# raywan-110/AdaQP

Hardware: NVIDIA H100
Metric: epochs_per_sec (higher is better)
Workload: dtype f32

## Files before the change

adaqp_b200/csrc/gemm.cu:

```cuda
#include <cuda.h>

#include "common.cuh"

namespace {

constexpr int kGemmThreads = 384;
constexpr int kBlockM = 128;
constexpr int kMaxN = 256;

__device__ __forceinline__ uint32_t smem_addr(const void *p) { return (uint32_t)__cvta_generic_to_shared(p); }

__device__ __forceinline__ void mbar_init(uint32_t bar, uint32_t count) {
    asm volatile("mbarrier.init.shared::cta.b64 [%0], %1;" ::"r"(bar), "r"(count) : "memory");
}
__device__ __forceinline__ void mbar_expect_tx(uint32_t bar, uint32_t bytes) {
    asm volatile("mbarrier.arrive.expect_tx.shared::cta.b64 _, [%0], %1;" ::"r"(bar), "r"(bytes) : "memory");
}
__device__ __forceinline__ void mbar_arrive(uint32_t bar) {
    asm volatile("mbarrier.arrive.shared::cta.b64 _, [%0];" ::"r"(bar) : "memory");
}
__device__ __forceinline__ void mbar_wait(uint32_t bar, uint32_t parity) {
    uint32_t done = 0;
    for (uint32_t spin = 0; spin < (1u << 26); ++spin) {
        asm volatile(
            "{\n"
            ".reg .pred p;\n"
            "mbarrier.try_wait.parity.shared::cta.b64 p, [%1], %2;\n"
            "selp.u32 %0, 1, 0, p;\n"
            "}\n" : "=r"(done) : "r"(bar), "r"(parity) : "memory");
        if (done) return;
    }
    __trap();
}
__device__ __forceinline__ void tma_load_2d(uint32_t dst, const CUtensorMap *map, int c0, int c1, uint32_t bar) {
    asm volatile("cp.async.bulk.tensor.2d.shared::cluster.global.tile.mbarrier::complete_tx::bytes [%0], [%1, {%2, %3}], [%4];"
                 ::"r"(dst), "l"(map), "r"(c0), "r"(c1), "r"(bar) : "memory");
}
__device__ __forceinline__ void wgmma_fence() { asm volatile("wgmma.fence.sync.aligned;" ::: "memory"); }
__device__ __forceinline__ void wgmma_commit() { asm volatile("wgmma.commit_group.sync.aligned;" ::: "memory"); }
__device__ __forceinline__ void wgmma_wait_all() { asm volatile("wgmma.wait_group.sync.aligned 0;" ::: "memory"); }

__device__ __forceinline__ uint64_t wgmma_desc(uint32_t saddr, uint32_t row_bytes) {
    uint64_t d = 0;
    d |= (uint64_t)((saddr >> 4) & 0x3FFF);
    d |= (uint64_t)1 << 16;
    d |= (uint64_t)((8u * row_bytes) >> 4) << 32;
    d |= (uint64_t)(row_bytes == 128 ? 1 : 2) << 62;
    return d;
}

__device__ __forceinline__ uint32_t swizzled(uint32_t r, uint32_t c, uint32_t row_bytes) {
    const uint32_t o = r * row_bytes + c * 4u;
    return o ^ (((o >> 7) & (row_bytes == 128 ? 7u : 3u)) << 4);
}

__device__ __forceinline__ void split_tf32(float x, uint32_t &hi, uint32_t &lo) {
    const float h = __uint_as_float(__float_as_uint(x) & 0xFFFFE000u);
    hi = __float_as_uint(h);
    lo = __float_as_uint(x - h);
}

template <int N> struct Wgmma;
template <> struct Wgmma<64> {
    static __device__ __forceinline__ void mma(float (&d)[32], const uint32_t (&a)[4], uint64_t b, uint32_t acc) {
        asm volatile(
            "{\n.reg .pred p;\nsetp.ne.b32 p, %37, 0;\n"
            "wgmma.mma_async.sync.aligned.m64n64k8.f32.tf32.tf32 {"
            "%0, %1, %2, %3, %4, %5, %6, %7, %8, %9, %10, %11, %12, %13, %14, %15, "
            "%16, %17, %18, %19, %20, %21, %22, %23, %24, %25, %26, %27, %28, %29, %30, %31"
            "}, {%32, %33, %34, %35}, %36, p, 1, 1;\n}\n"
            : "+f"(d[0]), "+f"(d[1]), "+f"(d[2]), "+f"(d[3]), "+f"(d[4]), "+f"(d[5]), "+f"(d[6]), "+f"(d[7]),
              "+f"(d[8]), "+f"(d[9]), "+f"(d[10]), "+f"(d[11]), "+f"(d[12]), "+f"(d[13]), "+f"(d[14]), "+f"(d[15]),
              "+f"(d[16]), "+f"(d[17]), "+f"(d[18]), "+f"(d[19]), "+f"(d[20]), "+f"(d[21]), "+f"(d[22]), "+f"(d[23]),
              "+f"(d[24]), "+f"(d[25]), "+f"(d[26]), "+f"(d[27]), "+f"(d[28]), "+f"(d[29]), "+f"(d[30]), "+f"(d[31])
            : "r"(a[0]), "r"(a[1]), "r"(a[2]), "r"(a[3]), "l"(b), "r"(acc));
    }
};
template <> struct Wgmma<128> {
    static __device__ __forceinline__ void mma(float (&d)[64], const uint32_t (&a)[4], uint64_t b, uint32_t acc) {
        asm volatile(
            "{\n.reg .pred p;\nsetp.ne.b32 p, %69, 0;\n"
            "wgmma.mma_async.sync.aligned.m64n128k8.f32.tf32.tf32 {"
            "%0, %1, %2, %3, %4, %5, %6, %7, %8, %9, %10, %11, %12, %13, %14, %15, "
            "%16, %17, %18, %19, %20, %21, %22, %23, %24, %25, %26, %27, %28, %29, %30, %31, "
            "%32, %33, %34, %35, %36, %37, %38, %39, %40, %41, %42, %43, %44, %45, %46, %47, "
            "%48, %49, %50, %51, %52, %53, %54, %55, %56, %57, %58, %59, %60, %61, %62, %63"
            "}, {%64, %65, %66, %67}, %68, p, 1, 1;\n}\n"
            : "+f"(d[0]), "+f"(d[1]), "+f"(d[2]), "+f"(d[3]), "+f"(d[4]), "+f"(d[5]), "+f"(d[6]), "+f"(d[7]),
              "+f"(d[8]), "+f"(d[9]), "+f"(d[10]), "+f"(d[11]), "+f"(d[12]), "+f"(d[13]), "+f"(d[14]), "+f"(d[15]),
              "+f"(d[16]), "+f"(d[17]), "+f"(d[18]), "+f"(d[19]), "+f"(d[20]), "+f"(d[21]), "+f"(d[22]), "+f"(d[23]),
              "+f"(d[24]), "+f"(d[25]), "+f"(d[26]), "+f"(d[27]), "+f"(d[28]), "+f"(d[29]), "+f"(d[30]), "+f"(d[31]),
              "+f"(d[32]), "+f"(d[33]), "+f"(d[34]), "+f"(d[35]), "+f"(d[36]), "+f"(d[37]), "+f"(d[38]), "+f"(d[39]),
              "+f"(d[40]), "+f"(d[41]), "+f"(d[42]), "+f"(d[43]), "+f"(d[44]), "+f"(d[45]), "+f"(d[46]), "+f"(d[47]),
              "+f"(d[48]), "+f"(d[49]), "+f"(d[50]), "+f"(d[51]), "+f"(d[52]), "+f"(d[53]), "+f"(d[54]), "+f"(d[55]),
              "+f"(d[56]), "+f"(d[57]), "+f"(d[58]), "+f"(d[59]), "+f"(d[60]), "+f"(d[61]), "+f"(d[62]), "+f"(d[63])
            : "r"(a[0]), "r"(a[1]), "r"(a[2]), "r"(a[3]), "l"(b), "r"(acc));
    }
};
template <> struct Wgmma<256> {
    static __device__ __forceinline__ void mma(float (&d)[128], const uint32_t (&a)[4], uint64_t b, uint32_t acc) {
        asm volatile(
            "{\n.reg .pred p;\nsetp.ne.b32 p, %133, 0;\n"
            "wgmma.mma_async.sync.aligned.m64n256k8.f32.tf32.tf32 {"
            "%0, %1, %2, %3, %4, %5, %6, %7, %8, %9, %10, %11, %12, %13, %14, %15, "
            "%16, %17, %18, %19, %20, %21, %22, %23, %24, %25, %26, %27, %28, %29, %30, %31, "
            "%32, %33, %34, %35, %36, %37, %38, %39, %40, %41, %42, %43, %44, %45, %46, %47, "
            "%48, %49, %50, %51, %52, %53, %54, %55, %56, %57, %58, %59, %60, %61, %62, %63, "
            "%64, %65, %66, %67, %68, %69, %70, %71, %72, %73, %74, %75, %76, %77, %78, %79, "
            "%80, %81, %82, %83, %84, %85, %86, %87, %88, %89, %90, %91, %92, %93, %94, %95, "
            "%96, %97, %98, %99, %100, %101, %102, %103, %104, %105, %106, %107, %108, %109, %110, %111, "
            "%112, %113, %114, %115, %116, %117, %118, %119, %120, %121, %122, %123, %124, %125, %126, %127"
            "}, {%128, %129, %130, %131}, %132, p, 1, 1;\n}\n"
            : "+f"(d[0]), "+f"(d[1]), "+f"(d[2]), "+f"(d[3]), "+f"(d[4]), "+f"(d[5]), "+f"(d[6]), "+f"(d[7]),
              "+f"(d[8]), "+f"(d[9]), "+f"(d[10]), "+f"(d[11]), "+f"(d[12]), "+f"(d[13]), "+f"(d[14]), "+f"(d[15]),
              "+f"(d[16]), "+f"(d[17]), "+f"(d[18]), "+f"(d[19]), "+f"(d[20]), "+f"(d[21]), "+f"(d[22]), "+f"(d[23]),
              "+f"(d[24]), "+f"(d[25]), "+f"(d[26]), "+f"(d[27]), "+f"(d[28]), "+f"(d[29]), "+f"(d[30]), "+f"(d[31]),
              "+f"(d[32]), "+f"(d[33]), "+f"(d[34]), "+f"(d[35]), "+f"(d[36]), "+f"(d[37]), "+f"(d[38]), "+f"(d[39]),
              "+f"(d[40]), "+f"(d[41]), "+f"(d[42]), "+f"(d[43]), "+f"(d[44]), "+f"(d[45]), "+f"(d[46]), "+f"(d[47]),
              "+f"(d[48]), "+f"(d[49]), "+f"(d[50]), "+f"(d[51]), "+f"(d[52]), "+f"(d[53]), "+f"(d[54]), "+f"(d[55]),
              "+f"(d[56]), "+f"(d[57]), "+f"(d[58]), "+f"(d[59]), "+f"(d[60]), "+f"(d[61]), "+f"(d[62]), "+f"(d[63]),
              "+f"(d[64]), "+f"(d[65]), "+f"(d[66]), "+f"(d[67]), "+f"(d[68]), "+f"(d[69]), "+f"(d[70]), "+f"(d[71]),
              "+f"(d[72]), "+f"(d[73]), "+f"(d[74]), "+f"(d[75]), "+f"(d[76]), "+f"(d[77]), "+f"(d[78]), "+f"(d[79]),
              "+f"(d[80]), "+f"(d[81]), "+f"(d[82]), "+f"(d[83]), "+f"(d[84]), "+f"(d[85]), "+f"(d[86]), "+f"(d[87]),
              "+f"(d[88]), "+f"(d[89]), "+f"(d[90]), "+f"(d[91]), "+f"(d[92]), "+f"(d[93]), "+f"(d[94]), "+f"(d[95]),
              "+f"(d[96]), "+f"(d[97]), "+f"(d[98]), "+f"(d[99]), "+f"(d[100]), "+f"(d[101]), "+f"(d[102]), "+f"(d[103]),
              "+f"(d[104]), "+f"(d[105]), "+f"(d[106]), "+f"(d[107]), "+f"(d[108]), "+f"(d[109]), "+f"(d[110]), "+f"(d[111]),
              "+f"(d[112]), "+f"(d[113]), "+f"(d[114]), "+f"(d[115]), "+f"(d[116]), "+f"(d[117]), "+f"(d[118]), "+f"(d[119]),
              "+f"(d[120]), "+f"(d[121]), "+f"(d[122]), "+f"(d[123]), "+f"(d[124]), "+f"(d[125]), "+f"(d[126]), "+f"(d[127])
            : "r"(a[0]), "r"(a[1]), "r"(a[2]), "r"(a[3]), "l"(b), "r"(acc));
    }
};

__device__ __forceinline__ void load_split_a(const uint8_t *tile, uint32_t row_bytes, int r, int c, uint32_t (&hi)[4],
                                             uint32_t (&lo)[4]) {
    split_tf32(*reinterpret_cast<const float *>(tile + swizzled(r, c, row_bytes)), hi[0], lo[0]);
    split_tf32(*reinterpret_cast<const float *>(tile + swizzled(r + 8, c, row_bytes)), hi[1], lo[1]);
    split_tf32(*reinterpret_cast<const float *>(tile + swizzled(r, c + 4, row_bytes)), hi[2], lo[2]);
    split_tf32(*reinterpret_cast<const float *>(tile + swizzled(r + 8, c + 4, row_bytes)), hi[3], lo[3]);
}

template <int KB>
struct GemmCfg {
    static constexpr int kStages = KB == 32 ? 2 : 4;
    static constexpr uint32_t kRowBytes = KB * 4;
    static constexpr uint32_t kATile = kBlockM * KB * 4;
    static constexpr uint32_t kBTile = kMaxN * KB * 4;
    static constexpr uint32_t kStageBytes = kATile + 2 * kBTile;
    static constexpr uint32_t kSmemBytes = kStages * kStageBytes + 1024 + 256;
};

template <int KB, int NM>
__global__ void __launch_bounds__(kGemmThreads, 1)
gemm_tf32x3_kernel(const __grid_constant__ CUtensorMap map_a, const __grid_constant__ CUtensorMap map_bhi,
                   const __grid_constant__ CUtensorMap map_blo, const float *__restrict__ bias,
                   float *__restrict__ C, int64_t ldc, int M, int N, int K) {
    using Cfg = GemmCfg<KB>;
    constexpr int kStages = Cfg::kStages;
    extern __shared__ uint8_t smem_raw[];
    const uint32_t base = (smem_addr(smem_raw) + 1023u) & ~1023u;
    const uint8_t *gen = smem_raw + (base - smem_addr(smem_raw));
    const uint32_t bars = base + kStages * Cfg::kStageBytes;
    auto bar_full = [&](int s) { return bars + 8u * s; };
    auto bar_empty = [&](int s) { return bars + 8u * (kStages + s); };

    const int wg = threadIdx.x >> 7;
    const int k_blocks = (K + KB - 1) / KB;
    const int tiles = (M + kBlockM - 1) / kBlockM;
    const uint32_t stage_tx = Cfg::kATile + 2u * (uint32_t)NM * KB * 4u;

    if (threadIdx.x == 0) {
        for (int s = 0; s < kStages; ++s) { mbar_init(bar_full(s), 1); mbar_init(bar_empty(s), 8); }
        asm volatile("fence.mbarrier_init.release.cluster;" ::: "memory");
    }
    __syncthreads();

    if (wg == 0) {
        if (threadIdx.x == 0) {
            int s = 0; uint32_t ph = 0;
            for (int t = blockIdx.x; t < tiles; t += gridDim.x) {
                for (int kb = 0; kb < k_blocks; ++kb) {
                    mbar_wait(bar_empty(s), ph ^ 1u);
                    const uint32_t st = base + s * Cfg::kStageBytes;
                    mbar_expect_tx(bar_full(s), stage_tx);
                    tma_load_2d(st, &map_a, kb * KB, t * kBlockM, bar_full(s));
                    tma_load_2d(st + Cfg::kATile, &map_bhi, kb * KB, 0, bar_full(s));
                    tma_load_2d(st + Cfg::kATile + Cfg::kBTile, &map_blo, kb * KB, 0, bar_full(s));
                    if (++s == kStages) { s = 0; ph ^= 1u; }
                }
            }
        }
        return;
    }
    const int tid = threadIdx.x - 128 * wg;
    const int warp = tid >> 5, lane = tid & 31, g = lane >> 2, q = lane & 3;
    const int r0 = (wg - 1) * 64 + warp * 16 + g;
    const bool vec2 = (ldc & 1) == 0 && (reinterpret_cast<uintptr_t>(C) & 7) == 0;
    float acc[NM / 2];
#pragma unroll
    for (int i = 0; i < NM / 2; ++i) acc[i] = 0.f;
    int s = 0; uint32_t ph = 0;
    for (int t = blockIdx.x; t < tiles; t += gridDim.x) {
        for (int kb = 0; kb < k_blocks; ++kb) {
            mbar_wait(bar_full(s), ph);
            const uint8_t *ta = gen + s * Cfg::kStageBytes;
            const uint32_t bhi = base + s * Cfg::kStageBytes + Cfg::kATile, blo = bhi + Cfg::kBTile;
#pragma unroll
            for (int k = 0; k < KB / 8; ++k) {
                uint32_t ahi[4], alo[4];
                load_split_a(ta, Cfg::kRowBytes, r0, k * 8 + q, ahi, alo);
                const uint64_t dhi = wgmma_desc(bhi + k * 32, Cfg::kRowBytes), dlo = wgmma_desc(blo + k * 32, Cfg::kRowBytes);
                wgmma_fence();
                Wgmma<NM>::mma(acc, alo, dhi, (kb | k) != 0);
                Wgmma<NM>::mma(acc, ahi, dlo, 1);
                Wgmma<NM>::mma(acc, ahi, dhi, 1);
                wgmma_commit();
                wgmma_wait_all();
            }
            __syncwarp();
            if (lane == 0) mbar_arrive(bar_empty(s));
            if (++s == kStages) { s = 0; ph ^= 1u; }
        }
#pragma unroll
        for (int j = 0; j < NM / 8; ++j) {
            const int col = j * 8 + 2 * q;
            const float b0 = (bias && col < N) ? __ldg(bias + col) : 0.f;
            const float b1 = (bias && col + 1 < N) ? __ldg(bias + col + 1) : 0.f;
#pragma unroll
            for (int h = 0; h < 2; ++h) {
                const int64_t row = (int64_t)t * kBlockM + r0 + 8 * h;
                if (row < M && col < N) {
                    float *p = C + row * ldc + col;
                    const float v0 = bias ? acc[4 * j + 2 * h] + b0 : acc[4 * j + 2 * h];
                    const float v1 = bias ? acc[4 * j + 2 * h + 1] + b1 : acc[4 * j + 2 * h + 1];
                    if (vec2 && col + 1 < N) {
                        *reinterpret_cast<float2 *>(p) = make_float2(v0, v1);
                    } else {
                        p[0] = v0;
                        if (col + 1 < N) p[1] = v1;
                    }
                }
            }
        }
    }
}

constexpr int kWgThreads = 384;
constexpr int kWgRows = 32;
constexpr int kWgStages = 3;
constexpr int kWgTileN = 128;
constexpr uint32_t kWgBox = kWgRows * 128;
constexpr uint32_t kWgDy = 4 * kWgBox;
constexpr uint32_t kWgX = 8 * kWgBox;
constexpr uint32_t kWgStageBytes = kWgDy + kWgX;
constexpr uint32_t kWgXt = kMaxN * 128;
constexpr uint32_t kWgSmemBytes = kWgStages * kWgStageBytes + 2 * kWgXt + 1024 + 256;

__device__ __forceinline__ void consumers_sync() { asm volatile("bar.sync 1, 256;" ::: "memory"); }

template <int NM>
__global__ void __launch_bounds__(kWgThreads, 1)
wgrad_tf32x3_kernel(const __grid_constant__ CUtensorMap map_dy, const __grid_constant__ CUtensorMap map_x,
                    float *__restrict__ partials, int M, int N, int K) {
    extern __shared__ uint8_t smem_raw[];
    const uint32_t base = (smem_addr(smem_raw) + 1023u) & ~1023u;
    uint8_t *gen = smem_raw + (base - smem_addr(smem_raw));
    const uint32_t xt_hi = base + kWgStages * kWgStageBytes, xt_lo = xt_hi + kWgXt;
    const uint32_t bars = xt_lo + kWgXt;
    auto bar_full = [&](int s) { return bars + 8u * s; };
    auto bar_empty = [&](int s) { return bars + 8u * (kWgStages + s); };

    const int wg = threadIdx.x >> 7;
    const int n0 = blockIdx.y * kWgTileN;
    const int n_left = (N - n0 + 31) / 32;
    const int n_chunks = n_left < 4 ? n_left : 4;
    const int k_chunks = (K + 31) / 32;
    const int blocks = (M + kWgRows - 1) / kWgRows;
    const int per = (blocks + gridDim.x - 1) / gridDim.x;
    const int b0 = blockIdx.x * per;
    const int b1 = (b0 + per < blocks) ? b0 + per : blocks;
    const uint32_t stage_tx = (uint32_t)(n_chunks + k_chunks) * kWgBox;

    if (threadIdx.x == 0) {
        for (int s = 0; s < kWgStages; ++s) { mbar_init(bar_full(s), 1); mbar_init(bar_empty(s), 8); }
        asm volatile("fence.mbarrier_init.release.cluster;" ::: "memory");
    }
    __syncthreads();

    if (wg == 0) {
        if (threadIdx.x == 0) {
            int s = 0; uint32_t ph = 0;
            for (int b = b0; b < b1; ++b) {
                mbar_wait(bar_empty(s), ph ^ 1u);
                const uint32_t st = base + s * kWgStageBytes;
                mbar_expect_tx(bar_full(s), stage_tx);
                for (int c = 0; c < n_chunks; ++c) tma_load_2d(st + c * kWgBox, &map_dy, n0 + c * 32, b * kWgRows, bar_full(s));
                for (int c = 0; c < k_chunks; ++c) tma_load_2d(st + kWgDy + c * kWgBox, &map_x, c * 32, b * kWgRows, bar_full(s));
                if (++s == kWgStages) { s = 0; ph ^= 1u; }
            }
        }
        return;
    }
    const int ctid = threadIdx.x - 128;
    const int tid = threadIdx.x - 128 * wg;
    const int warp = tid >> 5, lane = tid & 31, g = lane >> 2, q = lane & 3;
    const int nr = (wg - 1) * 64 + warp * 16 + g;
    const bool active = n0 + (wg - 1) * 64 < N;
    float acc[NM / 2];
#pragma unroll
    for (int i = 0; i < NM / 2; ++i) acc[i] = 0.f;
    int s = 0; uint32_t ph = 0;
    for (int b = b0; b < b1; ++b) {
        mbar_wait(bar_full(s), ph);
        const uint8_t *st = gen + s * kWgStageBytes;
        consumers_sync();
        for (int idx = ctid; idx < NM * kWgRows; idx += 256) {
            const int j = idx % NM, m = idx / NM;
            const float v = j < 32 * k_chunks
                ? *reinterpret_cast<const float *>(st + kWgDy + (j >> 5) * kWgBox + m * 128 + (j & 31) * 4) : 0.f;
            uint32_t h, l;
            split_tf32(v, h, l);
            const uint32_t o = swizzled(j, m, 128);
            *reinterpret_cast<uint32_t *>(gen + (xt_hi - base) + o) = h;
            *reinterpret_cast<uint32_t *>(gen + (xt_lo - base) + o) = l;
        }
        asm volatile("fence.proxy.async.shared::cta;" ::: "memory");
        consumers_sync();
        if (active) {
#pragma unroll
            for (int k = 0; k < kWgRows / 8; ++k) {
                uint32_t ahi[4], alo[4];
#pragma unroll
                for (int i = 0; i < 4; ++i) {
                    const int n = nr + 8 * (i & 1), m = 8 * k + q + 4 * (i >> 1);
                    split_tf32(*reinterpret_cast<const float *>(st + (n >> 5) * kWgBox + swizzled(m, n & 31, 128)), ahi[i], alo[i]);
                }
                const uint64_t dhi = wgmma_desc(xt_hi + k * 32, 128), dlo = wgmma_desc(xt_lo + k * 32, 128);
                wgmma_fence();
                Wgmma<NM>::mma(acc, alo, dhi, (b != b0) || (k != 0));
                Wgmma<NM>::mma(acc, ahi, dlo, 1);
                Wgmma<NM>::mma(acc, ahi, dhi, 1);
                wgmma_commit();
                wgmma_wait_all();
            }
        }
        __syncwarp();
        if (lane == 0) mbar_arrive(bar_empty(s));
        if (++s == kWgStages) { s = 0; ph ^= 1u; }
    }
    float *out = partials + (size_t)blockIdx.x * N * K;
#pragma unroll
    for (int j = 0; j < NM / 8; ++j) {
#pragma unroll
        for (int h = 0; h < 2; ++h) {
            const int n = n0 + nr + 8 * h;
#pragma unroll
            for (int e = 0; e < 2; ++e) {
                const int col = j * 8 + 2 * q + e;
                if (n < N && col < K) out[(size_t)n * K + col] = acc[4 * j + 2 * h + e];
            }
        }
    }
}

typedef CUresult (*EncodeTiledFn)(CUtensorMap *, CUtensorMapDataType, cuuint32_t, void *, const cuuint64_t *, const cuuint64_t *,
                                  const cuuint32_t *, const cuuint32_t *, CUtensorMapInterleave, CUtensorMapSwizzle,
                                  CUtensorMapL2promotion, CUtensorMapFloatOOBfill);

EncodeTiledFn encoder() {
    void *fn = nullptr;
    cudaDriverEntryPointQueryResult q;
    if (cudaGetDriverEntryPoint("cuTensorMapEncodeTiled", &fn, cudaEnableDefault, &q) != cudaSuccess) return nullptr;
    return q == cudaDriverEntryPointSuccess ? (EncodeTiledFn)fn : nullptr;
}

int make_tile_map(CUtensorMap *m, const float *base, int64_t rows, int64_t cols, int64_t ld, int box_rows,
                  CUtensorMapSwizzle swizzle, int box_cols) {
    EncodeTiledFn enc = encoder();
    ADAQP_REQUIRE(enc != nullptr, ADAQP_EINVAL, "cuTensorMapEncodeTiled not available from the driver");
    const cuuint64_t dims[2] = {(cuuint64_t)cols, (cuuint64_t)rows};
    const cuuint64_t strides[1] = {(cuuint64_t)ld * 4};
    const cuuint32_t box[2] = {(cuuint32_t)box_cols, (cuuint32_t)box_rows};
    const cuuint32_t estr[2] = {1, 1};
    const CUresult r = enc(m, CU_TENSOR_MAP_DATA_TYPE_FLOAT32, 2, (void *)base, dims, strides, box, estr, CU_TENSOR_MAP_INTERLEAVE_NONE,
                           swizzle, CU_TENSOR_MAP_L2_PROMOTION_L2_256B, CU_TENSOR_MAP_FLOAT_OOB_FILL_NONE);
    ADAQP_REQUIRE(r == CUDA_SUCCESS, ADAQP_EINVAL, "cuTensorMapEncodeTiled failed (%d)", (int)r);
    return 0;
}

inline int mma_n(int n) { return n <= 64 ? 64 : (n <= 128 ? 128 : 256); }

template <int KB, int NM>
int launch_gemm(const CUtensorMap &ma, const CUtensorMap &mh, const CUtensorMap &ml, const float *bias, float *C, int64_t ldc,
                int64_t M, int N, int K, int grid, cudaStream_t stream) {
    ADAQP_CUDA(cudaFuncSetAttribute(gemm_tf32x3_kernel<KB, NM>, cudaFuncAttributeMaxDynamicSharedMemorySize, (int)GemmCfg<KB>::kSmemBytes));
    gemm_tf32x3_kernel<KB, NM><<<grid, kGemmThreads, GemmCfg<KB>::kSmemBytes, stream>>>(ma, mh, ml, bias, C, ldc, (int)M, N, K);
    return adaqp_check_launch("gemm_tf32x3_kernel");
}

template <int NM>
int launch_wgrad(const CUtensorMap &my, const CUtensorMap &mx, float *partials, int64_t M, int N, int K, int grid, cudaStream_t stream) {
    ADAQP_CUDA(cudaFuncSetAttribute(wgrad_tf32x3_kernel<NM>, cudaFuncAttributeMaxDynamicSharedMemorySize, (int)kWgSmemBytes));
    const dim3 g(grid, (N + kWgTileN - 1) / kWgTileN);
    wgrad_tf32x3_kernel<NM><<<g, kWgThreads, kWgSmemBytes, stream>>>(my, mx, partials, (int)M, N, K);
    return adaqp_check_launch("wgrad_tf32x3_kernel");
}

}

extern "C" {

int adaqp_gemm_tf32x3_supported(int64_t M, int32_t N, int32_t K, int64_t lda, int64_t ldb, int64_t ldc) {
    if (M <= 0 || N <= 0 || K <= 0 || N > kMaxN || K > 4096) return 0;
    if ((lda & 3) || (ldb & 3) || lda < K || ldb < K || ldc < N) return 0;
    return 1;
}

int adaqp_gemm_tf32x3_f32(const float *A, int64_t lda, const float *Bt_hi, const float *Bt_lo, int64_t ldb,
                          const float *bias, int64_t M, int32_t N, int32_t K, float *C, int64_t ldc, void *stream) {
    ADAQP_REQUIRE(adaqp_gemm_tf32x3_supported(M, N, K, lda, ldb, ldc), ADAQP_ELIMIT,
                  "adaqp_gemm_tf32x3_f32: unsupported shape M=%lld N=%d K=%d lda=%lld ldb=%lld", (long long)M, N, K,
                  (long long)lda, (long long)ldb);
    ADAQP_REQUIRE(A && Bt_hi && Bt_lo && C, ADAQP_EINVAL, "adaqp_gemm_tf32x3_f32: null pointer");
    ADAQP_REQUIRE(((uintptr_t)A & 15) == 0 && ((uintptr_t)Bt_hi & 15) == 0 && ((uintptr_t)Bt_lo & 15) == 0, ADAQP_EALIGN,
                  "adaqp_gemm_tf32x3_f32: operands must be 16-byte aligned");
    ADAQP_REQUIRE(M < (1ll << 31), ADAQP_ELIMIT, "adaqp_gemm_tf32x3_f32: M too large");
    const int nm = mma_n(N);
    const int kb = adaqp_options().gemm_block_k == 32 ? 32 : 16;
    const CUtensorMapSwizzle sw = kb == 32 ? CU_TENSOR_MAP_SWIZZLE_128B : CU_TENSOR_MAP_SWIZZLE_64B;
    CUtensorMap ma, mh, ml;
    int rc = make_tile_map(&ma, A, M, K, lda, kBlockM, sw, kb);
    if (rc) return rc;
    rc = make_tile_map(&mh, Bt_hi, N, K, ldb, nm, sw, kb);
    if (rc) return rc;
    rc = make_tile_map(&ml, Bt_lo, N, K, ldb, nm, sw, kb);
    if (rc) return rc;
    const int sms = adaqp_sm_count() > 0 ? adaqp_sm_count() : 132;
    const int64_t tiles = (M + kBlockM - 1) / kBlockM;
    const int grid = (int)(tiles < sms ? tiles : sms);
    const cudaStream_t s = (cudaStream_t)stream;
    if (kb == 32) {
        if (nm == 64) return launch_gemm<32, 64>(ma, mh, ml, bias, C, ldc, M, N, K, grid, s);
        if (nm == 128) return launch_gemm<32, 128>(ma, mh, ml, bias, C, ldc, M, N, K, grid, s);
        return launch_gemm<32, 256>(ma, mh, ml, bias, C, ldc, M, N, K, grid, s);
    }
    if (nm == 64) return launch_gemm<16, 64>(ma, mh, ml, bias, C, ldc, M, N, K, grid, s);
    if (nm == 128) return launch_gemm<16, 128>(ma, mh, ml, bias, C, ldc, M, N, K, grid, s);
    return launch_gemm<16, 256>(ma, mh, ml, bias, C, ldc, M, N, K, grid, s);
}

int adaqp_wgrad_tf32x3_supported(int64_t M, int32_t N, int32_t K, int64_t ldy, int64_t ldx) {
    if (M <= 0 || N <= 0 || K <= 0 || N > kMaxN || K > kMaxN || M >= (1ll << 31)) return 0;
    if ((ldy & 3) || (ldx & 3) || ldy < N || ldx < K) return 0;
    return 1;
}

int adaqp_wgrad_tf32x3_grid(int64_t M) {
    const int sms = adaqp_sm_count() > 0 ? adaqp_sm_count() : 132;
    const int64_t blocks = (M + kWgRows - 1) / kWgRows;
    return (int)(blocks < sms ? (blocks < 1 ? 1 : blocks) : sms);
}

int adaqp_wgrad_tf32x3_f32(const float *dY, int64_t ldy, const float *X, int64_t ldx, int64_t M, int32_t N, int32_t K,
                           float *partials, int32_t grid, void *stream) {
    ADAQP_REQUIRE(adaqp_wgrad_tf32x3_supported(M, N, K, ldy, ldx), ADAQP_ELIMIT,
                  "adaqp_wgrad_tf32x3_f32: unsupported shape M=%lld N=%d K=%d", (long long)M, N, K);
    ADAQP_REQUIRE(dY && X && partials, ADAQP_EINVAL, "adaqp_wgrad_tf32x3_f32: null pointer");
    ADAQP_REQUIRE(((uintptr_t)dY & 15) == 0 && ((uintptr_t)X & 15) == 0, ADAQP_EALIGN, "adaqp_wgrad_tf32x3_f32: 16-byte alignment");
    ADAQP_REQUIRE(grid == adaqp_wgrad_tf32x3_grid(M), ADAQP_EINVAL, "adaqp_wgrad_tf32x3_f32: partials must hold adaqp_wgrad_tf32x3_grid(M) slices");
    CUtensorMap my, mx;
    int rc = make_tile_map(&my, dY, M, N, ldy, kWgRows, CU_TENSOR_MAP_SWIZZLE_128B, 32);
    if (rc) return rc;
    rc = make_tile_map(&mx, X, M, K, ldx, kWgRows, CU_TENSOR_MAP_SWIZZLE_NONE, 32);
    if (rc) return rc;
    const cudaStream_t s = (cudaStream_t)stream;
    const int nm = mma_n(K);
    if (nm == 64) return launch_wgrad<64>(my, mx, partials, M, N, K, grid, s);
    if (nm == 128) return launch_wgrad<128>(my, mx, partials, M, N, K, grid, s);
    return launch_wgrad<256>(my, mx, partials, M, N, K, grid, s);
}

}
```

Measured before the change: 8.654.

## Double-buffer wgrad X transpose and overlap async wgmma with next block staging

The wgrad kernel now keeps two transposed X buffers and ping-pongs between them. It issues each block's wgmma chain asynchronously and waits with wait_group 1, so the split/transpose of the next block overlaps the previous block's tensor-core work, and it releases the TMA stage earlier. Producer and consumer register budgets are rebalanced with setmaxnreg, and the stage count and smem size are sized per NM. The grid axes are swapped so N tiles vary fastest, which could change L2 reuse. This costs more shared memory (fewer stages for NM=256) and more registers for the prefetched A fragments.

```diff
diff --git a/adaqp_b200/csrc/gemm.cu b/adaqp_b200/csrc/gemm.cu
--- a/adaqp_b200/csrc/gemm.cu
+++ b/adaqp_b200/csrc/gemm.cu
@@ -38,7 +38,13 @@
 }
 __device__ __forceinline__ void wgmma_fence() { asm volatile("wgmma.fence.sync.aligned;" ::: "memory"); }
 __device__ __forceinline__ void wgmma_commit() { asm volatile("wgmma.commit_group.sync.aligned;" ::: "memory"); }
-__device__ __forceinline__ void wgmma_wait_all() { asm volatile("wgmma.wait_group.sync.aligned 0;" ::: "memory"); }
+template <int N>
+__device__ __forceinline__ void wgmma_wait() { asm volatile("wgmma.wait_group.sync.aligned %0;" ::"n"(N) : "memory"); }
+
+constexpr int kProducerRegs = 40;
+constexpr int kConsumerRegs = 232;
+__device__ __forceinline__ void producer_regs() { asm volatile("setmaxnreg.dec.sync.aligned.u32 %0;" ::"n"(kProducerRegs)); }
+__device__ __forceinline__ void consumer_regs() { asm volatile("setmaxnreg.inc.sync.aligned.u32 %0;" ::"n"(kConsumerRegs)); }
 
 __device__ __forceinline__ uint64_t wgmma_desc(uint32_t saddr, uint32_t row_bytes) {
     uint64_t d = 0;
@@ -214,7 +220,7 @@
                 Wgmma<NM>::mma(acc, ahi, dlo, 1);
                 Wgmma<NM>::mma(acc, ahi, dhi, 1);
                 wgmma_commit();
-                wgmma_wait_all();
+                wgmma_wait<0>();
             }
             __syncwarp();
             if (lane == 0) mbar_arrive(bar_empty(s));
@@ -246,14 +252,18 @@
 
 constexpr int kWgThreads = 384;
 constexpr int kWgRows = 32;
-constexpr int kWgStages = 3;
 constexpr int kWgTileN = 128;
 constexpr uint32_t kWgBox = kWgRows * 128;
 constexpr uint32_t kWgDy = 4 * kWgBox;
 constexpr uint32_t kWgX = 8 * kWgBox;
 constexpr uint32_t kWgStageBytes = kWgDy + kWgX;
-constexpr uint32_t kWgXt = kMaxN * 128;
-constexpr uint32_t kWgSmemBytes = kWgStages * kWgStageBytes + 2 * kWgXt + 1024 + 256;
+template <int NM>
+struct WgCfg {
+    static constexpr uint32_t kXt = NM * 128;
+    static constexpr int kStages = NM == 256 ? 2 : 3;
+    static constexpr uint32_t kSmemBytes = kStages * kWgStageBytes + 4 * kXt + 1024 + 256;
+    static_assert(kSmemBytes <= 227 * 1024, "wgrad_tf32x3_kernel: shared memory above the sm_90 per-block limit");
+};
 
 __device__ __forceinline__ void consumers_sync() { asm volatile("bar.sync 1, 256;" ::: "memory"); }
 
@@ -261,22 +271,24 @@
 __global__ void __launch_bounds__(kWgThreads, 1)
 wgrad_tf32x3_kernel(const __grid_constant__ CUtensorMap map_dy, const __grid_constant__ CUtensorMap map_x,
                     float *__restrict__ partials, int M, int N, int K) {
+    constexpr int kWgStages = WgCfg<NM>::kStages;
+    constexpr uint32_t kWgXt = WgCfg<NM>::kXt;
     extern __shared__ uint8_t smem_raw[];
     const uint32_t base = (smem_addr(smem_raw) + 1023u) & ~1023u;
     uint8_t *gen = smem_raw + (base - smem_addr(smem_raw));
-    const uint32_t xt_hi = base + kWgStages * kWgStageBytes, xt_lo = xt_hi + kWgXt;
-    const uint32_t bars = xt_lo + kWgXt;
+    const uint32_t xt_hi = base + kWgStages * kWgStageBytes;
+    const uint32_t bars = xt_hi + 4 * kWgXt;
     auto bar_full = [&](int s) { return bars + 8u * s; };
     auto bar_empty = [&](int s) { return bars + 8u * (kWgStages + s); };
 
     const int wg = threadIdx.x >> 7;
-    const int n0 = blockIdx.y * kWgTileN;
+    const int n0 = blockIdx.x * kWgTileN;
     const int n_left = (N - n0 + 31) / 32;
     const int n_chunks = n_left < 4 ? n_left : 4;
     const int k_chunks = (K + 31) / 32;
     const int blocks = (M + kWgRows - 1) / kWgRows;
-    const int per = (blocks + gridDim.x - 1) / gridDim.x;
-    const int b0 = blockIdx.x * per;
+    const int per = (blocks + gridDim.y - 1) / gridDim.y;
+    const int b0 = blockIdx.y * per;
     const int b1 = (b0 + per < blocks) ? b0 + per : blocks;
     const uint32_t stage_tx = (uint32_t)(n_chunks + k_chunks) * kWgBox;
 
@@ -287,6 +299,7 @@
     __syncthreads();
 
     if (wg == 0) {
+        producer_regs();
         if (threadIdx.x == 0) {
             int s = 0; uint32_t ph = 0;
             for (int b = b0; b < b1; ++b) {
@@ -300,18 +313,24 @@
         }
         return;
     }
+    consumer_regs();
     const int ctid = threadIdx.x - 128;
     const int tid = threadIdx.x - 128 * wg;
     const int warp = tid >> 5, lane = tid & 31, g = lane >> 2, q = lane & 3;
     const int nr = (wg - 1) * 64 + warp * 16 + g;
     const bool active = n0 + (wg - 1) * 64 < N;
+    constexpr int kSteps = kWgRows / 8;
     float acc[NM / 2];
 #pragma unroll
     for (int i = 0; i < NM / 2; ++i) acc[i] = 0.f;
+    uint32_t ahi0[kSteps][4], alo0[kSteps][4], ahi1[kSteps][4], alo1[kSteps][4];
     int s = 0; uint32_t ph = 0;
-    for (int b = b0; b < b1; ++b) {
+    auto block = [&](uint32_t (&ahi)[kSteps][4], uint32_t (&alo)[kSteps][4], int b) {
+        const uint32_t xoff = (uint32_t)((b - b0) & 1) * 2u * kWgXt;
+        const uint32_t xhi = xt_hi + xoff, xlo = xhi + kWgXt;
         mbar_wait(bar_full(s), ph);
         const uint8_t *st = gen + s * kWgStageBytes;
+        wgmma_wait<1>();
         consumers_sync();
         for (int idx = ctid; idx < NM * kWgRows; idx += 256) {
             const int j = idx % NM, m = idx / NM;
@@ -320,34 +339,42 @@
             uint32_t h, l;
             split_tf32(v, h, l);
             const uint32_t o = swizzled(j, m, 128);
-            *reinterpret_cast<uint32_t *>(gen + (xt_hi - base) + o) = h;
-            *reinterpret_cast<uint32_t *>(gen + (xt_lo - base) + o) = l;
-        }
+            *reinterpret_cast<uint32_t *>(gen + (xhi - base) + o) = h;
+            *reinterpret_cast<uint32_t *>(gen + (xlo - base) + o) = l;
+        }
+        if (active) {
+#pragma unroll
+            for (int k = 0; k < kSteps; ++k) {
+#pragma unroll
+                for (int i = 0; i < 4; ++i) {
+                    const int n = nr + 8 * (i & 1), m = 8 * k + q + 4 * (i >> 1);
+                    split_tf32(*reinterpret_cast<const float *>(st + (n >> 5) * kWgBox + swizzled(m, n & 31, 128)), ahi[k][i], alo[k][i]);
+                }
+            }
+        }
+        __syncwarp();
+        if (lane == 0) mbar_arrive(bar_empty(s));
+        if (++s == kWgStages) { s = 0; ph ^= 1u; }
         asm volatile("fence.proxy.async.shared::cta;" ::: "memory");
         consumers_sync();
         if (active) {
-#pragma unroll
-            for (int k = 0; k < kWgRows / 8; ++k) {
-                uint32_t ahi[4], alo[4];
-#pragma unroll
-                for (int i = 0; i < 4; ++i) {
-                    const int n = nr + 8 * (i & 1), m = 8 * k + q + 4 * (i >> 1);
-                    split_tf32(*reinterpret_cast<const float *>(st + (n >> 5) * kWgBox + swizzled(m, n & 31, 128)), ahi[i], alo[i]);
-                }
-                const uint64_t dhi = wgmma_desc(xt_hi + k * 32, 128), dlo = wgmma_desc(xt_lo + k * 32, 128);
-                wgmma_fence();
-                Wgmma<NM>::mma(acc, alo, dhi, (b != b0) || (k != 0));
-                Wgmma<NM>::mma(acc, ahi, dlo, 1);
-                Wgmma<NM>::mma(acc, ahi, dhi, 1);
-                wgmma_commit();
-                wgmma_wait_all();
-            }
-        }
-        __syncwarp();
-        if (lane == 0) mbar_arrive(bar_empty(s));
-        if (++s == kWgStages) { s = 0; ph ^= 1u; }
-    }
-    float *out = partials + (size_t)blockIdx.x * N * K;
+            wgmma_fence();
+#pragma unroll
+            for (int k = 0; k < kSteps; ++k) {
+                const uint64_t dhi = wgmma_desc(xhi + k * 32, 128), dlo = wgmma_desc(xlo + k * 32, 128);
+                Wgmma<NM>::mma(acc, alo[k], dhi, (b != b0) || (k != 0));
+                Wgmma<NM>::mma(acc, ahi[k], dlo, 1);
+                Wgmma<NM>::mma(acc, ahi[k], dhi, 1);
+            }
+            wgmma_commit();
+        }
+    };
+    for (int b = b0; b < b1; b += 2) {
+        block(ahi0, alo0, b);
+        if (b + 1 < b1) block(ahi1, alo1, b + 1);
+    }
+    wgmma_wait<0>();
+    float *out = partials + (size_t)blockIdx.y * N * K;
 #pragma unroll
     for (int j = 0; j < NM / 8; ++j) {
 #pragma unroll
@@ -399,9 +426,9 @@
 
 template <int NM>
 int launch_wgrad(const CUtensorMap &my, const CUtensorMap &mx, float *partials, int64_t M, int N, int K, int grid, cudaStream_t stream) {
-    ADAQP_CUDA(cudaFuncSetAttribute(wgrad_tf32x3_kernel<NM>, cudaFuncAttributeMaxDynamicSharedMemorySize, (int)kWgSmemBytes));
-    const dim3 g(grid, (N + kWgTileN - 1) / kWgTileN);
-    wgrad_tf32x3_kernel<NM><<<g, kWgThreads, kWgSmemBytes, stream>>>(my, mx, partials, (int)M, N, K);
+    ADAQP_CUDA(cudaFuncSetAttribute(wgrad_tf32x3_kernel<NM>, cudaFuncAttributeMaxDynamicSharedMemorySize, (int)WgCfg<NM>::kSmemBytes));
+    const dim3 g((N + kWgTileN - 1) / kWgTileN, grid);
+    wgrad_tf32x3_kernel<NM><<<g, kWgThreads, WgCfg<NM>::kSmemBytes, stream>>>(my, mx, partials, (int)M, N, K);
     return adaqp_check_launch("wgrad_tf32x3_kernel");
 }
 
```

Result: no change. 8.727, median of 6 (+0.8%).
